# nagadomi/nunif

Hardware: NVIDIA H100
Metric: waifu2x_input_megapixels_per_sec (higher is better)
Workload: dtype f16

## Files before the change

nunif_b200/csrc/swin_block.cu:

```cuda
#include "gemm_wgmma.cuh"
#include "swin_kernels.h"
#include "tmap.h"

namespace nb200 {

constexpr int FM_ROWS = 128, FM_STAGES = 5, FM_THREADS = GEMM_CONSUMER_THREADS + 128;
constexpr int FM_PRODUCER_REGS = 40, FM_CONSUMER_REGS = 232;

template <int C>
struct FmCfg {
    static constexpr int KB = C / 32;
    static constexpr int TILE = FM_ROWS * C * 2;
    static constexpr int STAGE = 128 * C;
    static constexpr int SMEM = 2 * TILE + FM_STAGES * STAGE + (2 * FM_STAGES + KB + 1) * 8 + 1024;
};

struct FmMaps {
    CUtensorMap x, att, wp, w1, w2, y, wy;
};

template <int K>
__device__ __forceinline__ float (&half96(float (&acc)[K], int h))[48] { return *reinterpret_cast<float(*)[48]>(&acc[48 * h]); }

__device__ __forceinline__ void wgmma_wait_n(int n) {
    if (n == 0) wgmma_wait<0>();
    else wgmma_wait<1>();
}

template <int C, bool PROJ, int CS>
__global__ void __launch_bounds__(FM_THREADS, 1) swin_mlp_fused_kernel(const __grid_constant__ FmMaps maps, const float* __restrict__ bp,
                                                                     const float* __restrict__ b1, const float* __restrict__ b2,
                                                                     const float* __restrict__ by) {
    using Cfg = FmCfg<C>;
    static_assert(CS % 16 == 0 && 2 * C * CS <= Cfg::STAGE && CS * 256 <= Cfg::TILE, "Wy must fit a ring stage, y the att tile");
    constexpr int KB = Cfg::KB, NP = (KB + 1) / 2, NH = 2 * C / 64, NHALF = C / 96;
    extern __shared__ uint8_t smem_dyn[];
    uint8_t* smem = reinterpret_cast<uint8_t*>((reinterpret_cast<uintptr_t>(smem_dyn) + 1023) & ~(uintptr_t)1023);
    uint8_t* sx = smem;
    uint8_t* satt = smem + Cfg::TILE;
    uint8_t* ring = smem + 2 * Cfg::TILE;
    uint64_t* full = reinterpret_cast<uint64_t*>(ring + FM_STAGES * Cfg::STAGE);
    uint64_t* empty = full + FM_STAGES;
    uint64_t* abar = empty + FM_STAGES;
    uint64_t* xbar = abar + KB;
    const int tid = threadIdx.x, warp = tid >> 5;
    const int row_base = blockIdx.x * FM_ROWS;
    if (tid == GEMM_CONSUMER_THREADS) {
        tma_prefetch_desc(&maps.x);
        tma_prefetch_desc(&maps.w1);
        tma_prefetch_desc(&maps.w2);
        if (CS) tma_prefetch_desc(&maps.wy);
        if (PROJ) {
            tma_prefetch_desc(&maps.att);
            tma_prefetch_desc(&maps.wp);
        }
        for (int s = 0; s < FM_STAGES; ++s) {
            mbar_init(&full[s], 1);
            mbar_init(&empty[s], 2);
        }
        for (int kb = 0; kb < KB; ++kb) mbar_init(&abar[kb], 1);
        mbar_init(xbar, 1);
        fence_barrier_init();
    }
    __syncthreads();

    if (warp >= GEMM_CONSUMER_THREADS / 32) {
        asm volatile("setmaxnreg.dec.sync.aligned.u32 %0;" ::"n"(FM_PRODUCER_REGS));
        if (warp == GEMM_CONSUMER_THREADS / 32 && elect_one()) {
            bool acts = false;
            auto load_acts = [&]() {
                asm volatile("griddepcontrol.wait;" ::: "memory");
                if (PROJ)
                    for (int kb = 0; kb < KB; ++kb) {
                        mbar_expect_tx(&abar[kb], FM_ROWS * 64);
                        tma_load_2d(&maps.att, &abar[kb], satt + kb * (FM_ROWS * 64), kb * 32, row_base);
                    }
                mbar_expect_tx(xbar, Cfg::TILE);
                for (int kb = 0; kb < KB; ++kb) tma_load_2d(&maps.x, xbar, sx + kb * (FM_ROWS * 64), kb * 32, row_base);
                acts = true;
            };
            int it = 0;
            auto push = [&](const CUtensorMap* m, int k0, int n0, int rows, int nbox) {
                if (it == FM_STAGES) load_acts();
                const int s = it % FM_STAGES;
                mbar_wait(&empty[s], ((it / FM_STAGES) & 1) ^ 1);
                mbar_expect_tx(&full[s], nbox * rows * 64);
                for (int b = 0; b < nbox; ++b) tma_load_2d(m, &full[s], ring + s * Cfg::STAGE + b * rows * 64, k0 + 32 * b, n0);
                ++it;
            };
            if (PROJ)
                for (int j = 0; j < NP; ++j) push(&maps.wp, 64 * j, 0, C, min(2, KB - 2 * j));
            push(&maps.w1, 0, 0, 64, KB);
            for (int hc = 0; hc < NH; ++hc) {
                if (hc + 1 < NH) push(&maps.w1, 0, (hc + 1) * 64, 64, KB);
                push(&maps.w2, hc * 64, 0, C, 2);
            }
            if (CS) push(&maps.wy, 0, 0, CS, KB);
            if (!acts) load_acts();
        }
        return;
    }

    asm volatile("setmaxnreg.inc.sync.aligned.u32 %0;" ::"n"(FM_CONSUMER_REGS));
    const int wg = tid >> 7, t = tid & 127;
    const int row0 = wg * 64 + (t >> 5) * 16 + ((t & 31) >> 2);
    const int cq = 2 * (t & 3);
    const uint32_t x_base = smem_u32(sx) + wg * 64 * 64, att_base = smem_u32(satt) + wg * 64 * 64;
    int it = 0, pending = 0;
    auto take = [&]() -> uint32_t {
        const int s = it % FM_STAGES;
        mbar_wait(&full[s], (it / FM_STAGES) & 1);
        return smem_u32(ring + s * Cfg::STAGE);
    };
    auto commit = [&]() {
        wgmma_commit();
        ++it;
        ++pending;
    };
    auto retire = [&](int n) {
        wgmma_wait_n(n);
#pragma unroll
        for (int k = 0; k < FM_STAGES; ++k)
            if (k < pending - n && t == 0) mbar_arrive(&empty[(it - pending + k) % FM_STAGES]);
        pending = min(pending, n);
    };

    if (PROJ) {
        float acc[C / 2];
#pragma unroll
        for (int j = 0; j < C / 2; ++j) acc[j] = 0.f;
        wgmma_fence_operands(acc);
#pragma unroll
        for (int j = 0; j < NP; ++j) {
            const uint32_t bb = take();
#pragma unroll
            for (int kb = 2 * j; kb < 2 * j + 2 && kb < KB; ++kb) mbar_wait(&abar[kb], 0);
            wgmma_fence();
#pragma unroll
            for (int kb = 2 * j; kb < 2 * j + 2 && kb < KB; ++kb) {
                const uint32_t a = att_base + kb * (FM_ROWS * 64), b = bb + (kb - 2 * j) * (C * 64);
#pragma unroll
                for (int s = 0; s < 2; ++s)
#pragma unroll
                    for (int h = 0; h < NHALF; ++h)
                        wgmma_f16<96>(half96(acc, h), make_kmajor_desc<64>(a + 32 * s), make_kmajor_desc<64>(b + h * 96 * 64 + 32 * s), 1u);
            }
            commit();
            retire(1);
        }
        retire(0);
        wgmma_fence_operands(acc);
        mbar_wait(xbar, 0);
#pragma unroll
        for (int j = 0; j < C / 8; ++j) {
            const int col = 8 * j + cq;
            const float2 bq = __ldg(reinterpret_cast<const float2*>(bp + col));
#pragma unroll
            for (int i = 0; i < 2; ++i) {
                __half2* p = reinterpret_cast<__half2*>(sx + sw64_off<FM_ROWS>(row0 + 8 * i, col));
                const float2 xv = __half22float2(*p);
                *p = __floats2half2_rn(xv.x + (acc[4 * j + 2 * i] + bq.x), xv.y + (acc[4 * j + 2 * i + 1] + bq.y));
            }
        }
        fence_async_smem();
        asm volatile("bar.sync %0, 128;" ::"r"(2 + wg) : "memory");
    } else {
        mbar_wait(xbar, 0);
    }

    float oacc[C / 2];
#pragma unroll
    for (int j = 0; j < C / 2; ++j) oacc[j] = 0.f;
    wgmma_fence_operands(oacc);
    float hacc[2][32];
    uint32_t af[4][4];
    auto fc1 = [&](float (&h)[32]) {
#pragma unroll
        for (int j = 0; j < 32; ++j) h[j] = 0.f;
        wgmma_fence_operands(h);
        const uint32_t bb = take();
        wgmma_fence();
#pragma unroll
        for (int kb = 0; kb < KB; ++kb) {
            const uint32_t a = x_base + kb * (FM_ROWS * 64), b = bb + kb * (64 * 64);
            wgmma_f16<64>(h, make_kmajor_desc<64>(a), make_kmajor_desc<64>(b), 1u);
            wgmma_f16<64>(h, make_kmajor_desc<64>(a + 32), make_kmajor_desc<64>(b + 32), 1u);
        }
        commit();
    };
    fc1(hacc[0]);
#pragma unroll
    for (int hc = 0; hc < NH; ++hc) {
        const int buf = hc & 1;
        if (hc + 1 < NH) fc1(hacc[buf ^ 1]);
        retire(hc + 1 < NH ? 1 : 0);
        wgmma_fence_operands(hacc[buf]);
#pragma unroll
        for (int kk = 0; kk < 4; ++kk)
#pragma unroll
            for (int q = 0; q < 4; ++q) {
                const int j = 2 * kk + (q >> 1), i = q & 1;
                const float2 bq = __ldg(reinterpret_cast<const float2*>(b1 + 64 * hc + 8 * j + cq));
                af[kk][q] = pack_half2(gelu_erf(hacc[buf][4 * j + 2 * i] + bq.x), gelu_erf(hacc[buf][4 * j + 2 * i + 1] + bq.y));
            }
        const uint32_t bb = take();
        wgmma_fence();
#pragma unroll
        for (int kb = 0; kb < 2; ++kb)
#pragma unroll
            for (int s = 0; s < 2; ++s)
#pragma unroll
                for (int h = 0; h < NHALF; ++h)
                    wgmma_f16_rs96(half96(oacc, h), af[2 * kb + s], make_kmajor_desc<64>(bb + kb * (C * 64) + h * 96 * 64 + 32 * s), 1u);
        commit();
    }
    retire(0);
    wgmma_fence_operands(oacc);
#pragma unroll
    for (int j = 0; j < C / 8; ++j) {
        const int col = 8 * j + cq;
        const float2 bq = __ldg(reinterpret_cast<const float2*>(b2 + col));
#pragma unroll
        for (int i = 0; i < 2; ++i) {
            __half2* p = reinterpret_cast<__half2*>(sx + sw64_off<FM_ROWS>(row0 + 8 * i, col));
            const float2 xv = __half22float2(*p);
            *p = __floats2half2_rn(xv.x + (oacc[4 * j + 2 * i] + bq.x), xv.y + (oacc[4 * j + 2 * i + 1] + bq.y));
        }
    }
    fence_async_smem();
    if constexpr (CS > 0) {
        asm volatile("bar.sync %0, 128;" ::"r"(2 + wg) : "memory");
        float yacc[CS / 2];
#pragma unroll
        for (int j = 0; j < CS / 2; ++j) yacc[j] = 0.f;
        wgmma_fence_operands(yacc);
        const uint32_t bb = take();
        wgmma_fence();
#pragma unroll
        for (int kb = 0; kb < KB; ++kb) {
            const uint32_t a = x_base + kb * (FM_ROWS * 64), b = bb + kb * (CS * 64);
            wgmma_f16<CS>(yacc, make_kmajor_desc<64>(a), make_kmajor_desc<64>(b), 1u);
            wgmma_f16<CS>(yacc, make_kmajor_desc<64>(a + 32), make_kmajor_desc<64>(b + 32), 1u);
        }
        commit();
        retire(0);
        wgmma_fence_operands(yacc);
#pragma unroll
        for (int j = 0; j < CS / 8; ++j) {
            const int col = 8 * j + cq;
            const float2 bq = __ldg(reinterpret_cast<const float2*>(by + col));
#pragma unroll
            for (int i = 0; i < 2; ++i) {
                __half2* p = reinterpret_cast<__half2*>(satt + (col >> 4) * (FM_ROWS * 32) + stage_off<16>(row0 + 8 * i, (col & 15) >> 3) +
                                                        (col & 7) * 2);
                *p = __floats2half2_rn(yacc[4 * j + 2 * i] + bq.x, yacc[4 * j + 2 * i + 1] + bq.y);
            }
        }
        fence_async_smem();
    }
    consumer_bar_sync();
    if (tid == 0) {
        if constexpr (CS > 0)
            for (int c = 0; c < CS / 16; ++c) tma_store_2d(&maps.y, satt + c * (FM_ROWS * 32), 16 * c, row_base);
        else
            for (int kb = 0; kb < KB; ++kb) tma_store_2d(&maps.x, sx + kb * (FM_ROWS * 64), kb * 32, row_base);
        tma_store_commit();
        tma_store_wait_read();
    }
}

static int map2d(CUtensorMap* m, const void* base, int cols, long long rows, int box_rows) {
    const cuuint64_t dims[2] = {(cuuint64_t)cols, (cuuint64_t)rows};
    const cuuint64_t strides[1] = {(cuuint64_t)cols * 2};
    const cuuint32_t box[2] = {32, (cuuint32_t)box_rows};
    return encode(m, base, 2, dims, strides, box, 64);
}

template <int C, bool PROJ, int CS = 0>
static int launch_mlp(cudaStream_t st, unsigned grid, const FmMaps& maps, const float* bp, const float* b1, const float* b2,
                      const float* by = nullptr) {
    if (ensure_dyn_smem((const void*)swin_mlp_fused_kernel<C, PROJ, CS>, FmCfg<C>::SMEM)) return 1;
    cudaLaunchConfig_t cfg = {};
    cfg.gridDim = dim3(grid); cfg.blockDim = dim3(FM_THREADS); cfg.dynamicSmemBytes = FmCfg<C>::SMEM;
    cfg.stream = st;
    cudaLaunchAttribute at[1];
    at[0].id = cudaLaunchAttributeProgrammaticStreamSerialization;
    at[0].val.programmaticStreamSerializationAllowed = 1;
    cfg.attrs = at; cfg.numAttrs = 1;
    NB_CUDA(cudaLaunchKernelEx(&cfg, swin_mlp_fused_kernel<C, PROJ, CS>, maps, bp, b1, b2, by));
    NB_LAUNCHED();
    return 0;
}

int swin_mlp_fused(cudaStream_t st, __half* x, const __half* att, long long T, int C, const __half* wp, const float* bp,
                   const __half* w1, const float* b1, const __half* w2, const float* b2, __half* y, int cs, const __half* wy,
                   const float* by) {
    NB_CHECK(x && w1 && b1 && w2 && b2 && (!att || (wp && bp)) && (!y || (att && wy && by)), "null pointer");
    NB_CHECK(C == 96 || C == 192, "C must be 96 or 192");
    NB_CHECK(!y || (C == 192 && cs == 48) || (C == 96 && cs == 16), "y: cs must be 48 at C = 192 and 16 at C = 96");
    NB_CHECK(T > 0 && T < (1LL << 31), "token count out of range");
    FmMaps maps;
    memset(&maps, 0, sizeof(maps));
    if (map2d(&maps.x, x, C, T, FM_ROWS)) return 1;
    if (att && (map2d(&maps.att, att, C, T, FM_ROWS) || map2d(&maps.wp, wp, C, C, C))) return 1;
    if (map2d(&maps.w1, w1, C, 2 * C, 64) || map2d(&maps.w2, w2, 2 * C, C, C)) return 1;
    if (y) {
        if (map2d(&maps.wy, wy, C, cs, cs)) return 1;
        const cuuint64_t dims[2] = {(cuuint64_t)cs, (cuuint64_t)T};
        const cuuint64_t strides[1] = {(cuuint64_t)cs * 2};
        const cuuint32_t box[2] = {16, FM_ROWS};
        if (encode(&maps.y, y, 2, dims, strides, box, 32)) return 1;
    }
    const double Td = (double)T;
    ProfScope ps(st, PC_FUSED_MLP, Td * C * 2 * (C * ((att ? 1 : 0) + 4) + (y ? cs : 0)), Td * C * 2 * (att ? 2 : 1),
                 Td * (y ? cs : C) * 2);
    const unsigned grid = (unsigned)((T + FM_ROWS - 1) / FM_ROWS);
    if (rec_on()) {
        char line[96];
        snprintf(line, sizeof(line), "swin_mlp,%lld,%d,%d,%d", T, C, att ? 1 : 0, y ? cs : 0);
        rec_append(line);
    }
    if (y) return C == 96 ? launch_mlp<96, true, 16>(st, grid, maps, bp, b1, b2, by) : launch_mlp<192, true, 48>(st, grid, maps, bp, b1, b2, by);
    if (C == 96) return att ? launch_mlp<96, true>(st, grid, maps, bp, b1, b2) : launch_mlp<96, false>(st, grid, maps, bp, b1, b2);
    return att ? launch_mlp<192, true>(st, grid, maps, bp, b1, b2) : launch_mlp<192, false>(st, grid, maps, bp, b1, b2);
}

}

using namespace nb200;

extern "C" int nb200_swin_mlp_fused_f16(void* x, const void* att, long long T, int C, const void* wp, const float* bp,
                                        const void* w1, const float* b1, const void* w2, const float* b2, void* stream) {
    return swin_mlp_fused((cudaStream_t)stream, (__half*)x, (const __half*)att, T, C, (const __half*)wp, bp, (const __half*)w1, b1,
                          (const __half*)w2, b2, nullptr, 0, nullptr, nullptr);
}

extern "C" int nb200_swin_mlp_fused_y_f16(void* x, const void* att, long long T, int C, const void* wp, const float* bp,
                                          const void* w1, const float* b1, const void* w2, const float* b2, void* y, int cs,
                                          const void* wy, const float* by, void* stream) {
    NB_CHECK(y, "null pointer");
    return swin_mlp_fused((cudaStream_t)stream, (__half*)x, (const __half*)att, T, C, (const __half*)wp, bp, (const __half*)w1, b1,
                          (const __half*)w2, b2, (__half*)y, cs, (const __half*)wy, by);
}

extern "C" int nb200_swin_attn_fused_f16(const void* x, const void* wqkv, const float* bqkv, const float* bias_table, void* att,
                                         int B, int H, int W, int C, int shift, void* stream) {
    NB_CHECK(bias_table, "null pointer");
    cudaStream_t st = (cudaStream_t)stream;
    float* frag = nullptr;
    NB_CUDA(cudaMallocAsync((void**)&frag, BIAS_FRAG_FLOATS * sizeof(float), st));
    int rc = build_bias_frag(st, bias_table, frag);
    if (!rc) rc = swin_attn_fused(st, (const __half*)x, (const __half*)wqkv, bqkv, frag, (__half*)att, B, H, W, C, shift);
    cudaFreeAsync(frag, st);
    return rc;
}
```

Baseline: 74.74.

## Make fused Swin MLP kernel persistent with overlapped tile output stores

Converts the fused MLP kernel into a persistent kernel that launches at most one block per SM and loops over 128-row tiles. The producer warp now issues the TMA store of the previous tile's output and prefetches the next tile's attention activations while weight stages stream, using new afree/oready mbarriers. An opaque volatile zero load keeps the compiler from hoisting per-tile address computations and blowing up registers. This removes per-block launch and prologue cost and overlaps output stores with compute, but it serialises activation reuse within a block and may lose parallelism when the tile count barely exceeds the SM count.

```diff
diff --git a/nunif_b200/csrc/swin_block.cu b/nunif_b200/csrc/swin_block.cu
--- a/nunif_b200/csrc/swin_block.cu
+++ b/nunif_b200/csrc/swin_block.cu
@@ -1,3 +1,4 @@
+#include <algorithm>
 #include "gemm_wgmma.cuh"
 #include "swin_kernels.h"
 #include "tmap.h"
@@ -12,7 +13,7 @@
     static constexpr int KB = C / 32;
     static constexpr int TILE = FM_ROWS * C * 2;
     static constexpr int STAGE = 128 * C;
-    static constexpr int SMEM = 2 * TILE + FM_STAGES * STAGE + (2 * FM_STAGES + KB + 1) * 8 + 1024;
+    static constexpr int SMEM = 2 * TILE + FM_STAGES * STAGE + (2 * FM_STAGES + KB + 4) * 8 + 1024;
 };
 
 struct FmMaps {
@@ -22,18 +23,25 @@
 template <int K>
 __device__ __forceinline__ float (&half96(float (&acc)[K], int h))[48] { return *reinterpret_cast<float(*)[48]>(&acc[48 * h]); }
 
+__device__ __forceinline__ int opaque_zero(const uint32_t* zero) {
+    int v;
+    asm volatile("ld.volatile.shared.u32 %0, [%1];" : "=r"(v) : "r"(smem_u32(zero)));
+    return v;
+}
+
 __device__ __forceinline__ void wgmma_wait_n(int n) {
     if (n == 0) wgmma_wait<0>();
     else wgmma_wait<1>();
 }
 
 template <int C, bool PROJ, int CS>
-__global__ void __launch_bounds__(FM_THREADS, 1) swin_mlp_fused_kernel(const __grid_constant__ FmMaps maps, const float* __restrict__ bp,
-                                                                     const float* __restrict__ b1, const float* __restrict__ b2,
-                                                                     const float* __restrict__ by) {
+__global__ void __launch_bounds__(FM_THREADS, 1) swin_mlp_fused_kernel(const __grid_constant__ FmMaps maps, const float* __restrict__ bp_,
+                                                                     const float* __restrict__ b1_, const float* __restrict__ b2_,
+                                                                     const float* __restrict__ by_, int ntiles) {
     using Cfg = FmCfg<C>;
     static_assert(CS % 16 == 0 && 2 * C * CS <= Cfg::STAGE && CS * 256 <= Cfg::TILE, "Wy must fit a ring stage, y the att tile");
     constexpr int KB = Cfg::KB, NP = (KB + 1) / 2, NH = 2 * C / 64, NHALF = C / 96;
+    static_assert(2 * NH > FM_STAGES, "the next tile's activations are loaded between this tile's W1 / W2 stages");
     extern __shared__ uint8_t smem_dyn[];
     uint8_t* smem = reinterpret_cast<uint8_t*>((reinterpret_cast<uintptr_t>(smem_dyn) + 1023) & ~(uintptr_t)1023);
     uint8_t* sx = smem;
@@ -43,13 +51,19 @@
     uint64_t* empty = full + FM_STAGES;
     uint64_t* abar = empty + FM_STAGES;
     uint64_t* xbar = abar + KB;
+    uint64_t* afree = xbar + 1;
+    uint64_t* oready = afree + 1;
+    uint32_t* zero = reinterpret_cast<uint32_t*>(oready + 1);
     const int tid = threadIdx.x, warp = tid >> 5;
-    const int row_base = blockIdx.x * FM_ROWS;
+    const int my_tiles = (ntiles - 1 - (int)blockIdx.x) / (int)gridDim.x + 1;
     if (tid == GEMM_CONSUMER_THREADS) {
         tma_prefetch_desc(&maps.x);
         tma_prefetch_desc(&maps.w1);
         tma_prefetch_desc(&maps.w2);
-        if (CS) tma_prefetch_desc(&maps.wy);
+        if (CS) {
+            tma_prefetch_desc(&maps.wy);
+            tma_prefetch_desc(&maps.y);
+        }
         if (PROJ) {
             tma_prefetch_desc(&maps.att);
             tma_prefetch_desc(&maps.wp);
@@ -60,6 +74,9 @@
         }
         for (int kb = 0; kb < KB; ++kb) mbar_init(&abar[kb], 1);
         mbar_init(xbar, 1);
+        mbar_init(afree, 2);
+        mbar_init(oready, 2);
+        *zero = 0;
         fence_barrier_init();
     }
     __syncthreads();
@@ -67,205 +84,245 @@
     if (warp >= GEMM_CONSUMER_THREADS / 32) {
         asm volatile("setmaxnreg.dec.sync.aligned.u32 %0;" ::"n"(FM_PRODUCER_REGS));
         if (warp == GEMM_CONSUMER_THREADS / 32 && elect_one()) {
-            bool acts = false;
-            auto load_acts = [&]() {
-                asm volatile("griddepcontrol.wait;" ::: "memory");
-                if (PROJ)
-                    for (int kb = 0; kb < KB; ++kb) {
-                        mbar_expect_tx(&abar[kb], FM_ROWS * 64);
-                        tma_load_2d(&maps.att, &abar[kb], satt + kb * (FM_ROWS * 64), kb * 32, row_base);
-                    }
+            auto row_of = [&](int k) { return ((int)blockIdx.x + k * (int)gridDim.x) * FM_ROWS; };
+            auto load_att = [&](int row) {
+                for (int kb = 0; kb < KB; ++kb) {
+                    mbar_expect_tx(&abar[kb], FM_ROWS * 64);
+                    tma_load_2d(&maps.att, &abar[kb], satt + kb * (FM_ROWS * 64), kb * 32, row);
+                }
+            };
+            auto load_x = [&](int row) {
                 mbar_expect_tx(xbar, Cfg::TILE);
-                for (int kb = 0; kb < KB; ++kb) tma_load_2d(&maps.x, xbar, sx + kb * (FM_ROWS * 64), kb * 32, row_base);
-                acts = true;
+                for (int kb = 0; kb < KB; ++kb) tma_load_2d(&maps.x, xbar, sx + kb * (FM_ROWS * 64), kb * 32, row);
+            };
+            auto store_out = [&](int k) {
+                mbar_wait(oready, k & 1);
+                const int row = row_of(k);
+                if constexpr (CS > 0)
+                    for (int c = 0; c < CS / 16; ++c) tma_store_2d(&maps.y, satt + c * (FM_ROWS * 32), 16 * c, row);
+                else
+                    for (int kb = 0; kb < KB; ++kb) tma_store_2d(&maps.x, sx + kb * (FM_ROWS * 64), kb * 32, row);
+                tma_store_commit();
+                tma_store_wait_read();
             };
             int it = 0;
-            auto push = [&](const CUtensorMap* m, int k0, int n0, int rows, int nbox) {
-                if (it == FM_STAGES) load_acts();
-                const int s = it % FM_STAGES;
-                mbar_wait(&empty[s], ((it / FM_STAGES) & 1) ^ 1);
-                mbar_expect_tx(&full[s], nbox * rows * 64);
-                for (int b = 0; b < nbox; ++b) tma_load_2d(m, &full[s], ring + s * Cfg::STAGE + b * rows * 64, k0 + 32 * b, n0);
-                ++it;
-            };
-            if (PROJ)
-                for (int j = 0; j < NP; ++j) push(&maps.wp, 64 * j, 0, C, min(2, KB - 2 * j));
-            push(&maps.w1, 0, 0, 64, KB);
-            for (int hc = 0; hc < NH; ++hc) {
-                if (hc + 1 < NH) push(&maps.w1, 0, (hc + 1) * 64, 64, KB);
-                push(&maps.w2, hc * 64, 0, C, 2);
+            for (int k = 0; k < my_tiles; ++k) {
+                int ti = 0;
+                auto push = [&](const CUtensorMap* m, int k0, int n0, int rows, int nbox) {
+                    if (ti == FM_STAGES) {
+                        if (k == 0) {
+                            asm volatile("griddepcontrol.wait;" ::: "memory");
+                            if (PROJ) load_att(row_of(k));
+                        } else {
+                            store_out(k - 1);
+                            if (PROJ && CS > 0) load_att(row_of(k));
+                        }
+                        load_x(row_of(k));
+                    }
+                    if (PROJ && CS == 0 && ti == NP + FM_STAGES && k + 1 < my_tiles) {
+                        mbar_wait(afree, k & 1);
+                        load_att(row_of(k + 1));
+                    }
+                    const int s = it % FM_STAGES;
+                    mbar_wait(&empty[s], ((it / FM_STAGES) & 1) ^ 1);
+                    mbar_expect_tx(&full[s], nbox * rows * 64);
+                    for (int b = 0; b < nbox; ++b) tma_load_2d(m, &full[s], ring + s * Cfg::STAGE + b * rows * 64, k0 + 32 * b, n0);
+                    ++it;
+                    ++ti;
+                };
+                if (PROJ)
+                    for (int j = 0; j < NP; ++j) push(&maps.wp, 64 * j, 0, C, min(2, KB - 2 * j));
+                push(&maps.w1, 0, 0, 64, KB);
+                for (int hc = 0; hc < NH; ++hc) {
+                    if (hc + 1 < NH) push(&maps.w1, 0, (hc + 1) * 64, 64, KB);
+                    push(&maps.w2, hc * 64, 0, C, 2);
+                }
+                if (CS) push(&maps.wy, 0, 0, CS, KB);
             }
-            if (CS) push(&maps.wy, 0, 0, CS, KB);
-            if (!acts) load_acts();
+            store_out(my_tiles - 1);
         }
         return;
     }
-
-    asm volatile("setmaxnreg.inc.sync.aligned.u32 %0;" ::"n"(FM_CONSUMER_REGS));
-    const int wg = tid >> 7, t = tid & 127;
-    const int row0 = wg * 64 + (t >> 5) * 16 + ((t & 31) >> 2);
-    const int cq = 2 * (t & 3);
-    const uint32_t x_base = smem_u32(sx) + wg * 64 * 64, att_base = smem_u32(satt) + wg * 64 * 64;
-    int it = 0, pending = 0;
-    auto take = [&]() -> uint32_t {
-        const int s = it % FM_STAGES;
-        mbar_wait(&full[s], (it / FM_STAGES) & 1);
-        return smem_u32(ring + s * Cfg::STAGE);
-    };
-    auto commit = [&]() {
-        wgmma_commit();
-        ++it;
-        ++pending;
-    };
-    auto retire = [&](int n) {
-        wgmma_wait_n(n);
-#pragma unroll
-        for (int k = 0; k < FM_STAGES; ++k)
-            if (k < pending - n && t == 0) mbar_arrive(&empty[(it - pending + k) % FM_STAGES]);
-        pending = min(pending, n);
-    };
-
-    if (PROJ) {
-        float acc[C / 2];
-#pragma unroll
-        for (int j = 0; j < C / 2; ++j) acc[j] = 0.f;
-        wgmma_fence_operands(acc);
-#pragma unroll
-        for (int j = 0; j < NP; ++j) {
-            const uint32_t bb = take();
-#pragma unroll
-            for (int kb = 2 * j; kb < 2 * j + 2 && kb < KB; ++kb) mbar_wait(&abar[kb], 0);
-            wgmma_fence();
-#pragma unroll
-            for (int kb = 2 * j; kb < 2 * j + 2 && kb < KB; ++kb) {
-                const uint32_t a = att_base + kb * (FM_ROWS * 64), b = bb + (kb - 2 * j) * (C * 64);
-#pragma unroll
-                for (int s = 0; s < 2; ++s)
-#pragma unroll
-                    for (int h = 0; h < NHALF; ++h)
-                        wgmma_f16<96>(half96(acc, h), make_kmajor_desc<64>(a + 32 * s), make_kmajor_desc<64>(b + h * 96 * 64 + 32 * s), 1u);
+    {
+        asm volatile("setmaxnreg.inc.sync.aligned.u32 %0;" ::"n"(FM_CONSUMER_REGS));
+        const int wg = tid >> 7, t = tid & 127;
+        int it = 0, pending = 0;
+        auto take = [&]() -> uint32_t {
+            const int s = it % FM_STAGES;
+            mbar_wait(&full[s], (it / FM_STAGES) & 1);
+            return smem_u32(ring + s * Cfg::STAGE);
+        };
+        auto commit = [&]() {
+            wgmma_commit();
+            ++it;
+            ++pending;
+        };
+        auto retire = [&](int n) {
+            wgmma_wait_n(n);
+#pragma unroll
+            for (int k = 0; k < FM_STAGES; ++k)
+                if (k < pending - n && t == 0) mbar_arrive(&empty[(it - pending + k) % FM_STAGES]);
+            pending = min(pending, n);
+        };
+
+#pragma unroll 1
+        for (int k = 0; k < my_tiles; ++k) {
+            const uint32_t ph = k & 1;
+            const int z = opaque_zero(zero);
+            auto frag_rc = [&](int& r0, int& c0) {
+                const int u = t + opaque_zero(zero);
+                r0 = wg * 64 + (u >> 5) * 16 + ((u & 31) >> 2);
+                c0 = 2 * (u & 3);
+            };
+            const int cqh = 2 * ((t + z) & 3);
+            uint8_t* const sx = smem + z;
+            uint8_t* const satt = sx + Cfg::TILE;
+            const uint32_t x_base = smem_u32(sx) + wg * 64 * 64, att_base = smem_u32(satt) + wg * 64 * 64;
+            const float* const bp = bp_ + z;
+            const float* const b1 = b1_ + z;
+            const float* const b2 = b2_ + z;
+            const float* const by = by_ + z;
+            if (PROJ) {
+                float acc[C / 2];
+#pragma unroll
+                for (int j = 0; j < C / 2; ++j) acc[j] = 0.f;
+                wgmma_fence_operands(acc);
+#pragma unroll
+                for (int j = 0; j < NP; ++j) {
+                    const uint32_t bb = take();
+#pragma unroll
+                    for (int kb = 2 * j; kb < 2 * j + 2 && kb < KB; ++kb) mbar_wait(&abar[kb], ph);
+                    wgmma_fence();
+#pragma unroll
+                    for (int kb = 2 * j; kb < 2 * j + 2 && kb < KB; ++kb) {
+                        const uint32_t a = att_base + kb * (FM_ROWS * 64), b = bb + (kb - 2 * j) * (C * 64);
+#pragma unroll
+                        for (int s = 0; s < 2; ++s)
+#pragma unroll
+                            for (int h = 0; h < NHALF; ++h)
+                                wgmma_f16<96>(half96(acc, h), make_kmajor_desc<64>(a + 32 * s), make_kmajor_desc<64>(b + h * 96 * 64 + 32 * s), 1u);
+                    }
+                    commit();
+                    retire(1);
+                }
+                retire(0);
+                wgmma_fence_operands(acc);
+                if (CS == 0 && t == 0) mbar_arrive(afree);
+                mbar_wait(xbar, ph);
+                int row0, cq;
+                frag_rc(row0, cq);
+#pragma unroll
+                for (int j = 0; j < C / 8; ++j) {
+                    const int col = 8 * j + cq;
+                    const float2 bq = __ldg(reinterpret_cast<const float2*>(bp + col));
+#pragma unroll
+                    for (int i = 0; i < 2; ++i) {
+                        __half2* p = reinterpret_cast<__half2*>(sx + sw64_off<FM_ROWS>(row0 + 8 * i, col));
+                        const float2 xv = __half22float2(*p);
+                        *p = __floats2half2_rn(xv.x + (acc[4 * j + 2 * i] + bq.x), xv.y + (acc[4 * j + 2 * i + 1] + bq.y));
+                    }
+                }
+                fence_async_smem();
+                asm volatile("bar.sync %0, 128;" ::"r"(2 + wg) : "memory");
+            } else {
+                mbar_wait(xbar, ph);
             }
-            commit();
-            retire(1);
+
+            float oacc[C / 2];
+#pragma unroll
+            for (int j = 0; j < C / 2; ++j) oacc[j] = 0.f;
+            wgmma_fence_operands(oacc);
+            float hacc[2][32];
+            uint32_t af[4][4];
+            auto fc1 = [&](float (&h)[32]) {
+#pragma unroll
+                for (int j = 0; j < 32; ++j) h[j] = 0.f;
+                wgmma_fence_operands(h);
+                const uint32_t bb = take();
+                wgmma_fence();
+#pragma unroll
+                for (int kb = 0; kb < KB; ++kb) {
+                    const uint32_t a = x_base + kb * (FM_ROWS * 64), b = bb + kb * (64 * 64);
+                    wgmma_f16<64>(h, make_kmajor_desc<64>(a), make_kmajor_desc<64>(b), 1u);
+                    wgmma_f16<64>(h, make_kmajor_desc<64>(a + 32), make_kmajor_desc<64>(b + 32), 1u);
+                }
+                commit();
+            };
+            fc1(hacc[0]);
+#pragma unroll
+            for (int hc = 0; hc < NH; ++hc) {
+                const int buf = hc & 1;
+                if (hc + 1 < NH) fc1(hacc[buf ^ 1]);
+                retire(hc + 1 < NH ? 1 : 0);
+                wgmma_fence_operands(hacc[buf]);
+#pragma unroll
+                for (int kk = 0; kk < 4; ++kk)
+#pragma unroll
+                    for (int q = 0; q < 4; ++q) {
+                        const int j = 2 * kk + (q >> 1), i = q & 1;
+                        const float2 bq = __ldg(reinterpret_cast<const float2*>(b1 + 64 * hc + 8 * j + cqh));
+                        af[kk][q] = pack_half2(gelu_erf(hacc[buf][4 * j + 2 * i] + bq.x), gelu_erf(hacc[buf][4 * j + 2 * i + 1] + bq.y));
+                    }
+                const uint32_t bb = take();
+                wgmma_fence();
+#pragma unroll
+                for (int kb = 0; kb < 2; ++kb)
+#pragma unroll
+                    for (int s = 0; s < 2; ++s)
+#pragma unroll
+                        for (int h = 0; h < NHALF; ++h)
+                            wgmma_f16_rs96(half96(oacc, h), af[2 * kb + s], make_kmajor_desc<64>(bb + kb * (C * 64) + h * 96 * 64 + 32 * s), 1u);
+                commit();
+            }
+            retire(0);
+            wgmma_fence_operands(oacc);
+            int row0, cq;
+            frag_rc(row0, cq);
+#pragma unroll
+            for (int j = 0; j < C / 8; ++j) {
+                const int col = 8 * j + cq;
+                const float2 bq = __ldg(reinterpret_cast<const float2*>(b2 + col));
+#pragma unroll
+                for (int i = 0; i < 2; ++i) {
+                    __half2* p = reinterpret_cast<__half2*>(sx + sw64_off<FM_ROWS>(row0 + 8 * i, col));
+                    const float2 xv = __half22float2(*p);
+                    *p = __floats2half2_rn(xv.x + (oacc[4 * j + 2 * i] + bq.x), xv.y + (oacc[4 * j + 2 * i + 1] + bq.y));
+                }
+            }
+            fence_async_smem();
+            if constexpr (CS > 0) {
+                asm volatile("bar.sync %0, 128;" ::"r"(2 + wg) : "memory");
+                float yacc[CS / 2];
+#pragma unroll
+                for (int j = 0; j < CS / 2; ++j) yacc[j] = 0.f;
+                wgmma_fence_operands(yacc);
+                const uint32_t bb = take();
+                wgmma_fence();
+#pragma unroll
+                for (int kb = 0; kb < KB; ++kb) {
+                    const uint32_t a = x_base + kb * (FM_ROWS * 64), b = bb + kb * (CS * 64);
+                    wgmma_f16<CS>(yacc, make_kmajor_desc<64>(a), make_kmajor_desc<64>(b), 1u);
+                    wgmma_f16<CS>(yacc, make_kmajor_desc<64>(a + 32), make_kmajor_desc<64>(b + 32), 1u);
+                }
+                commit();
+                retire(0);
+                wgmma_fence_operands(yacc);
+#pragma unroll
+                for (int j = 0; j < CS / 8; ++j) {
+                    const int col = 8 * j + cq;
+                    const float2 bq = __ldg(reinterpret_cast<const float2*>(by + col));
+#pragma unroll
+                    for (int i = 0; i < 2; ++i) {
+                        __half2* p = reinterpret_cast<__half2*>(satt + (col >> 4) * (FM_ROWS * 32) + stage_off<16>(row0 + 8 * i, (col & 15) >> 3) +
+                                                                (col & 7) * 2);
+                        *p = __floats2half2_rn(yacc[4 * j + 2 * i] + bq.x, yacc[4 * j + 2 * i + 1] + bq.y);
+                    }
+                }
+                fence_async_smem();
+            }
+            asm volatile("bar.sync %0, 128;" ::"r"(2 + wg) : "memory");
+            if (t == 0) mbar_arrive(oready);
         }
-        retire(0);
-        wgmma_fence_operands(acc);
-        mbar_wait(xbar, 0);
-#pragma unroll
-        for (int j = 0; j < C / 8; ++j) {
-            const int col = 8 * j + cq;
-            const float2 bq = __ldg(reinterpret_cast<const float2*>(bp + col));
-#pragma unroll
-            for (int i = 0; i < 2; ++i) {
-                __half2* p = reinterpret_cast<__half2*>(sx + sw64_off<FM_ROWS>(row0 + 8 * i, col));
-                const float2 xv = __half22float2(*p);
-                *p = __floats2half2_rn(xv.x + (acc[4 * j + 2 * i] + bq.x), xv.y + (acc[4 * j + 2 * i + 1] + bq.y));
-            }
-        }
-        fence_async_smem();
-        asm volatile("bar.sync %0, 128;" ::"r"(2 + wg) : "memory");
-    } else {
-        mbar_wait(xbar, 0);
-    }
-
-    float oacc[C / 2];
-#pragma unroll
-    for (int j = 0; j < C / 2; ++j) oacc[j] = 0.f;
-    wgmma_fence_operands(oacc);
-    float hacc[2][32];
-    uint32_t af[4][4];
-    auto fc1 = [&](float (&h)[32]) {
-#pragma unroll
-        for (int j = 0; j < 32; ++j) h[j] = 0.f;
-        wgmma_fence_operands(h);
-        const uint32_t bb = take();
-        wgmma_fence();
-#pragma unroll
-        for (int kb = 0; kb < KB; ++kb) {
-            const uint32_t a = x_base + kb * (FM_ROWS * 64), b = bb + kb * (64 * 64);
-            wgmma_f16<64>(h, make_kmajor_desc<64>(a), make_kmajor_desc<64>(b), 1u);
-            wgmma_f16<64>(h, make_kmajor_desc<64>(a + 32), make_kmajor_desc<64>(b + 32), 1u);
-        }
-        commit();
-    };
-    fc1(hacc[0]);
-#pragma unroll
-    for (int hc = 0; hc < NH; ++hc) {
-        const int buf = hc & 1;
-        if (hc + 1 < NH) fc1(hacc[buf ^ 1]);
-        retire(hc + 1 < NH ? 1 : 0);
-        wgmma_fence_operands(hacc[buf]);
-#pragma unroll
-        for (int kk = 0; kk < 4; ++kk)
-#pragma unroll
-            for (int q = 0; q < 4; ++q) {
-                const int j = 2 * kk + (q >> 1), i = q & 1;
-                const float2 bq = __ldg(reinterpret_cast<const float2*>(b1 + 64 * hc + 8 * j + cq));
-                af[kk][q] = pack_half2(gelu_erf(hacc[buf][4 * j + 2 * i] + bq.x), gelu_erf(hacc[buf][4 * j + 2 * i + 1] + bq.y));
-            }
-        const uint32_t bb = take();
-        wgmma_fence();
-#pragma unroll
-        for (int kb = 0; kb < 2; ++kb)
-#pragma unroll
-            for (int s = 0; s < 2; ++s)
-#pragma unroll
-                for (int h = 0; h < NHALF; ++h)
-                    wgmma_f16_rs96(half96(oacc, h), af[2 * kb + s], make_kmajor_desc<64>(bb + kb * (C * 64) + h * 96 * 64 + 32 * s), 1u);
-        commit();
-    }
-    retire(0);
-    wgmma_fence_operands(oacc);
-#pragma unroll
-    for (int j = 0; j < C / 8; ++j) {
-        const int col = 8 * j + cq;
-        const float2 bq = __ldg(reinterpret_cast<const float2*>(b2 + col));
-#pragma unroll
-        for (int i = 0; i < 2; ++i) {
-            __half2* p = reinterpret_cast<__half2*>(sx + sw64_off<FM_ROWS>(row0 + 8 * i, col));
-            const float2 xv = __half22float2(*p);
-            *p = __floats2half2_rn(xv.x + (oacc[4 * j + 2 * i] + bq.x), xv.y + (oacc[4 * j + 2 * i + 1] + bq.y));
-        }
-    }
-    fence_async_smem();
-    if constexpr (CS > 0) {
-        asm volatile("bar.sync %0, 128;" ::"r"(2 + wg) : "memory");
-        float yacc[CS / 2];
-#pragma unroll
-        for (int j = 0; j < CS / 2; ++j) yacc[j] = 0.f;
-        wgmma_fence_operands(yacc);
-        const uint32_t bb = take();
-        wgmma_fence();
-#pragma unroll
-        for (int kb = 0; kb < KB; ++kb) {
-            const uint32_t a = x_base + kb * (FM_ROWS * 64), b = bb + kb * (CS * 64);
-            wgmma_f16<CS>(yacc, make_kmajor_desc<64>(a), make_kmajor_desc<64>(b), 1u);
-            wgmma_f16<CS>(yacc, make_kmajor_desc<64>(a + 32), make_kmajor_desc<64>(b + 32), 1u);
-        }
-        commit();
-        retire(0);
-        wgmma_fence_operands(yacc);
-#pragma unroll
-        for (int j = 0; j < CS / 8; ++j) {
-            const int col = 8 * j + cq;
-            const float2 bq = __ldg(reinterpret_cast<const float2*>(by + col));
-#pragma unroll
-            for (int i = 0; i < 2; ++i) {
-                __half2* p = reinterpret_cast<__half2*>(satt + (col >> 4) * (FM_ROWS * 32) + stage_off<16>(row0 + 8 * i, (col & 15) >> 3) +
-                                                        (col & 7) * 2);
-                *p = __floats2half2_rn(yacc[4 * j + 2 * i] + bq.x, yacc[4 * j + 2 * i + 1] + bq.y);
-            }
-        }
-        fence_async_smem();
-    }
-    consumer_bar_sync();
-    if (tid == 0) {
-        if constexpr (CS > 0)
-            for (int c = 0; c < CS / 16; ++c) tma_store_2d(&maps.y, satt + c * (FM_ROWS * 32), 16 * c, row_base);
-        else
-            for (int kb = 0; kb < KB; ++kb) tma_store_2d(&maps.x, sx + kb * (FM_ROWS * 64), kb * 32, row_base);
-        tma_store_commit();
-        tma_store_wait_read();
     }
 }
 
@@ -277,17 +334,18 @@
 }
 
 template <int C, bool PROJ, int CS = 0>
-static int launch_mlp(cudaStream_t st, unsigned grid, const FmMaps& maps, const float* bp, const float* b1, const float* b2,
+static int launch_mlp(cudaStream_t st, long long ntiles, const FmMaps& maps, const float* bp, const float* b1, const float* b2,
                       const float* by = nullptr) {
     if (ensure_dyn_smem((const void*)swin_mlp_fused_kernel<C, PROJ, CS>, FmCfg<C>::SMEM)) return 1;
     cudaLaunchConfig_t cfg = {};
-    cfg.gridDim = dim3(grid); cfg.blockDim = dim3(FM_THREADS); cfg.dynamicSmemBytes = FmCfg<C>::SMEM;
+    cfg.gridDim = dim3((unsigned)std::min<long long>(ntiles, device_sm_count()));
+    cfg.blockDim = dim3(FM_THREADS); cfg.dynamicSmemBytes = FmCfg<C>::SMEM;
     cfg.stream = st;
     cudaLaunchAttribute at[1];
     at[0].id = cudaLaunchAttributeProgrammaticStreamSerialization;
     at[0].val.programmaticStreamSerializationAllowed = 1;
     cfg.attrs = at; cfg.numAttrs = 1;
-    NB_CUDA(cudaLaunchKernelEx(&cfg, swin_mlp_fused_kernel<C, PROJ, CS>, maps, bp, b1, b2, by));
+    NB_CUDA(cudaLaunchKernelEx(&cfg, swin_mlp_fused_kernel<C, PROJ, CS>, maps, bp, b1, b2, by, (int)ntiles));
     NB_LAUNCHED();
     return 0;
 }
@@ -314,15 +372,15 @@
     const double Td = (double)T;
     ProfScope ps(st, PC_FUSED_MLP, Td * C * 2 * (C * ((att ? 1 : 0) + 4) + (y ? cs : 0)), Td * C * 2 * (att ? 2 : 1),
                  Td * (y ? cs : C) * 2);
-    const unsigned grid = (unsigned)((T + FM_ROWS - 1) / FM_ROWS);
+    const long long ntiles = (T + FM_ROWS - 1) / FM_ROWS;
     if (rec_on()) {
         char line[96];
         snprintf(line, sizeof(line), "swin_mlp,%lld,%d,%d,%d", T, C, att ? 1 : 0, y ? cs : 0);
         rec_append(line);
     }
-    if (y) return C == 96 ? launch_mlp<96, true, 16>(st, grid, maps, bp, b1, b2, by) : launch_mlp<192, true, 48>(st, grid, maps, bp, b1, b2, by);
-    if (C == 96) return att ? launch_mlp<96, true>(st, grid, maps, bp, b1, b2) : launch_mlp<96, false>(st, grid, maps, bp, b1, b2);
-    return att ? launch_mlp<192, true>(st, grid, maps, bp, b1, b2) : launch_mlp<192, false>(st, grid, maps, bp, b1, b2);
+    if (y) return C == 96 ? launch_mlp<96, true, 16>(st, ntiles, maps, bp, b1, b2, by) : launch_mlp<192, true, 48>(st, ntiles, maps, bp, b1, b2, by);
+    if (C == 96) return att ? launch_mlp<96, true>(st, ntiles, maps, bp, b1, b2) : launch_mlp<96, false>(st, ntiles, maps, bp, b1, b2);
+    return att ? launch_mlp<192, true>(st, ntiles, maps, bp, b1, b2) : launch_mlp<192, false>(st, ntiles, maps, bp, b1, b2);
 }
 
 }
```

Result: no change. 75.37, median of 6 (+0.8%).
